# matwilso/generative_models

Hardware: AMD Instinct MI355X
Metric: ddpm_train_images_per_sec (higher is better)
Workload: dtype fp16_fwd+bf16_bwd; 1 GPU; DDPM train step, 3x32x32, SimpleUnet C=128, 2048 images per GPU, T=1000 (BASELINE.json configs[2]); key=cfg2, global_batch=2048, parallelism=dp1

## Files before the change

### generative_models_amd/diffusion/simple_unet.py

```python
import math
import os
from collections import OrderedDict

import torch
from torch import nn

from .. import ops

MAX_TIMESTEPS = 256


def _res_names(prefix, cin, cout, emb):
    out = [
        (f"{prefix}.in_layers.0.weight", (cin,)), (f"{prefix}.in_layers.0.bias", (cin,)),
        (f"{prefix}.in_layers.2.weight", (cout, cin, 3, 3)), (f"{prefix}.in_layers.2.bias", (cout,)),
        (f"{prefix}.emb_layers.1.weight", (cout, emb)), (f"{prefix}.emb_layers.1.bias", (cout,)),
        (f"{prefix}.out_layers.0.weight", (cout,)), (f"{prefix}.out_layers.0.bias", (cout,)),
        (f"{prefix}.out_layers.3.weight", (cout, cout, 3, 3)), (f"{prefix}.out_layers.3.bias", (cout,)),
    ]
    if cin != cout:
        out += [(f"{prefix}.skip_connection.weight", (cout, cin, 1, 1)), (f"{prefix}.skip_connection.bias", (cout,))]
    return out


# ... 608 lines not shown
                ds, dgp, dbp = ops.gn_silu_bwd(da, s, *gn[2:], dadd1=dskip, dadd2=add2, dxsum=ssum)
            if grads:
                ops.colsum(dgp, gw[i * C:(i + 1) * C], defer=True); ops.colsum(dbp, gb[i * C:(i + 1) * C], defer=True)
            outs.append((ds, ssum))
        return outs

    def prepare_forward(self, dev=None):
        if self._packs_stale or self._packed_version != self._version_sum():
            self._repack()
        dev = self.flat_params.device if dev is None else dev
        self._freq_table(MAX_TIMESTEPS, dev)
        self._freq_table(4, dev)

    def forward_hip(self, x, logsnr, guide=None, cond_w=None, ctx=None, want_nu=False):
        if want_nu and not self.learn_var:
            raise ValueError("forward_hip: want_nu on a network without the variance head (learn_var)")
        if self._packs_stale or self._packed_version != self._version_sum():
            self._repack()
        P, C, T = self._pv, self.channels, self.act_dtype
        B, cin, H, W = x.shape
        if cin != self.in_channels or H % 4 or W % 4:
            raise ValueError(f"input {tuple(x.shape)}: need {self.in_channels} channels and H, W divisible by 4")
        x = ops.aligned(x.float())
        logsnr, guide, cond_w = ops.aligned(logsnr), ops.aligned(guide), ops.aligned(cond_w)
        if ops.EMB_SIDE and ops.WGRAD_STREAM and x.is_cuda and not torch.cuda.is_current_stream_capturing():
            box = []
            self._on_side(lambda: box.append(self._embed_fwd(logsnr, guide, cond_w, ctx)), tuple(t for t in (logsnr, guide, cond_w) if t is not None))
            emb_all = box[0]
            self._emb_pending = emb_all
        else:
            emb_all = self._embed_fwd(logsnr, guide, cond_w, ctx)
        H2, W2, H4, W4 = H // 2, W // 2, H // 4, W // 4
        t0 = ops.stem_fwd(x, P["down.seq.0.conv.weight"], P["down.seq.0.conv.bias"], C, T)
        t1 = self._res_fwd("down.seq.1", [t0], emb_all, 0, ctx)
        t2 = self._res_fwd("down.seq.2", [t1], emb_all, 1, ctx)
        t3 = self._conv([t2], self._packs["down.seq.3.conv"][0], C, 3, ops.STRIDE2, (H2, W2),
                            bias=P["down.seq.3.conv.bias"])
        t4 = self._res_fwd("down.seq.4", [t3], emb_all, 2, ctx)
        t5 = self._res_fwd("down.seq.5", [t4], emb_all, 3, ctx)
        t6 = self._conv([t5], self._packs["down.seq.6.conv"][0], C, 3, ops.STRIDE2, (H4, W4),
                            bias=P["down.seq.6.conv.bias"])
        t7 = self._res_fwd("turn", [t6], emb_all, 4, ctx)
        if self.attention:
            t7 = self._attn_fwd(t7, ctx)
        u0r = self._res_fwd("up.seq.0.0", [t7, t6], emb_all, 5, ctx)
        u0 = self._upsample_conv("up.seq.0.1.conv", u0r, (H2, W2))
        u1 = self._res_fwd("up.seq.1", [u0, t5], emb_all, 6, ctx)
        u2 = self._res_fwd("up.seq.2", [u1, t4], emb_all, 7, ctx)
        u3r = self._res_fwd("up.seq.3.0", [u2, t3], emb_all, 8, ctx)
        u3 = self._upsample_conv("up.seq.3.1.conv", u3r, (H, W))
        u4 = self._res_fwd("up.seq.4", [u3, t2], emb_all, 9, ctx)
        u5 = self._res_fwd("up.seq.5", [u4, t1], emb_all, 10, ctx)
        u6 = self._res_fwd("up.seq.6", [u5, t0], emb_all, 11, ctx)
        ao, mo, ro = ops.gn_silu_fwd(u6, P["out.0.weight"], P["out.0.bias"], self._g1)
        out = ops.head_fwd(ao, P["out.2.weight"], P["out.2.bias"])
        if ctx is not None:
            ctx["net"] = (x, t2, t5, u0r, u3r, u6, ao, mo, ro)
            ctx["dims"] = (B, H, W)
        if want_nu:
            rows = B if want_nu is True else int(want_nu)
            if not 1 <= rows <= B:
                raise ValueError(f"forward_hip: want_nu = {want_nu} rows of a batch of {B}")
            return out, ops.head_fwd(ao if rows == B else ao[:rows], P["out_var.weight"], P["out_var.bias"])
        return out

    def grad_buckets(self):
        names = [n for n, _ in self._inventory]
        def rng(pred):
            return self.arena_range([n for n in names if pred(n)])
        late = ("up.seq.4", "up.seq.5", "up.seq.6", "out.", "out_var.")
        mid = ("up.seq.0", "up.seq.1", "up.seq.2", "up.seq.3")
        emb = ("time_embed", "cond_w_embed", "guide_embed")
        is_emb = lambda n: n.startswith(emb) or ".emb_layers." in n or n.endswith(".in_layers.2.bias")
        b0 = rng(lambda n: n.startswith(late) and not is_emb(n))
        b1 = rng(lambda n: n.startswith(mid) and not is_emb(n))
        b2 = rng(lambda n: (n.startswith("down.") or n.startswith("turn.") or n.startswith("attn.")) and not is_emb(n))
        b3 = rng(is_emb)
        buckets = [b0, b1, b2, b3]
        assert sorted(buckets)[0][0] == 0 and sorted(buckets)[-1][1] == self._arena_size
        srt = sorted(buckets)
        assert all(srt[i][1] == srt[i + 1][0] for i in range(3)), "gradient buckets must tile the arena"
        return buckets

    def backward_hip(self, ctx, dout, on_grads_ready=None, join_side_before_ready=True, want_dx=False, dnu=None):
        if ops.WGRAD_CUS > 0 and ops.WGRAD_STREAM and dout.is_cuda and self._cu_part is None and not (
                torch.distributed.is_available() and torch.distributed.is_initialized() and torch.distributed.get_world_size() > 1):
            full = ops.get_cu_limit()
            self._cu_part = (full, min(ops.WGRAD_CUS, full - 8))
            ops.set_cu_limit(full - self._cu_part[1])
            try:
                return self.backward_hip(ctx, dout, on_grads_ready, join_side_before_ready, want_dx, dnu)
            finally:
                ops.set_cu_limit(full)
                self._cu_part = None
        if dnu is not None and not self.learn_var:
            raise ValueError("backward_hip: dnu on a network without the variance head (learn_var)")
        if dnu is not None and tuple(dnu.shape) != tuple(dout.shape):
            raise ValueError(f"backward_hip: dnu has shape {tuple(dnu.shape)}, dout {tuple(dout.shape)}")
        join = self._join_side if (on_grads_ready is not None and join_side_before_ready) else None
        dt0 = self._backward_schedule(ctx, ops.aligned(dout.float()), True, on_grads_ready, join,
                                      dnu=None if dnu is None else ops.aligned(dnu.float()))
        return ops.stem_dgrad(dt0, self._pv["down.seq.0.conv.weight"]) if want_dx else None

    def input_vjp_hip(self, ctx, r):
        x = ctx["net"][0]
        if tuple(r.shape) != tuple(x.shape):
            raise ValueError(f"input_vjp_hip: r has shape {tuple(r.shape)}, the network output {tuple(x.shape)}")
        dt0 = self._backward_schedule(ctx, ops.aligned(r.float()), False)
        return ops.stem_dgrad(dt0, self._pv["down.seq.0.conv.weight"])

    def _backward_schedule(self, ctx, dout, grads, ready=None, join=None, dnu=None):
        P, G, C, T = self._pv, self._gv, self.channels, self.compute_dtype
        B, H, W = ctx["dims"]
        H2, W2 = H // 2, W // 2
        x, t2, t5, u0r, u3r, u6, ao, mo, ro = ctx["net"]
        dev = dout.device
        demb_all = torch.empty((B, 12 * C), device=dev, dtype=torch.float32) if grads else None
        pair = grads and ready is None
        ready = ready if ready is not None else (lambda k: None)
        join = join if join is not None else (lambda: None)
        res = lambda name, d, dsum, blk, extra=None, defer=False: self._res_bwd(name, ctx, d, dsum, demb_all, blk, extra_add=extra, grads=grads,
                                                                               defer_skip=defer and pair)

        def bucket_done(k):
            if grads:
                ops.flush_colsums(); join()
                ready(k)

        def up(name, d, dsum, src):
            if grads:
                ops.colsum(dsum, G[name + ".bias"], defer=True)
                self._upsample_wgrad(name, d, src)
            dsrc = self._upsample_dgrad(name, d)
            return dsrc, (ops.chansum(dsrc) if grads else None)

        def down(name, d, dsum, src, hw, skip):
            if grads:
                ops.colsum(dsum, G[name + ".bias"], defer=True)
                self._wgrad(d, [src], 3, ops.STRIDE2, G[name + ".weight"])
            dsrc = self._conv([d], self._packs[name][1], C, 3, ops.TRANSPOSED2, hw, residual=skip)
            return dsrc, (ops.chansum(dsrc) if grads else None)

        if grads:
            o = self._offsets["out.2.weight"]
            nhead = self.in_channels * C * 9
            assert self._offsets["out.2.bias"] == o + (nhead + 3) // 4 * 4 == o + nhead
            self._on_side(lambda: ops.head_wgrad(dout, ao, self.flat_grads[o:o + nhead + self.in_channels]), (dout, ao))
        dao = ops.head_dgrad(dout, P["out.2.weight"], T)
        if dnu is None and grads and self.learn_var:
            self.flat_grads[self._offsets["out_var.weight"]:].zero_()
        if dnu is not None:
            if grads:
                ov = self._offsets["out_var.weight"]
                assert self._offsets["out_var.bias"] == ov + nhead
                self._on_side(lambda: ops.head_wgrad(dnu, ao, self.flat_grads[ov:ov + nhead + self.in_channels]), (dnu, ao))
            ops.add_into(dao, ops.head_dgrad(dnu, P["out_var.weight"], T))
        s6 = torch.empty((B, C), device=dev, dtype=torch.float32) if grads else None
        du6, dgp, dbp = ops.gn_silu_bwd(dao, u6, P["out.0.weight"], P["out.0.bias"], mo, ro, dxsum=s6)
        if grads:
            ops.colsum(dgp, G["out.0.weight"], defer=True); ops.colsum(dbp, G["out.0.bias"], defer=True)

        (du5, s5), (dt0a, _) = res("up.seq.6", du6, s6, 11, defer=True)
        (du4, s4), (dt1a, _) = res("up.seq.5", du5, s5, 10, defer=True)
        (du3, s3), (dt2a, _) = res("up.seq.4", du4, s4, 9)
        bucket_done(0)
        du3r, s3r = up("up.seq.3.1.conv", du3, s3, u3r)
        (du2, s2), (dt3a, _) = res("up.seq.3.0", du3r, s3r, 8, defer=True)
        (du1, s1), (dt4a, _) = res("up.seq.2", du2, s2, 7, defer=True)
        (du0, s0), (dt5a, _) = res("up.seq.1", du1, s1, 6)
        du0r, s0r = up("up.seq.0.1.conv", du0, s0, u0r)
        (dt7, s7), (dt6a, _) = res("up.seq.0.0", du0r, s0r, 5)
        if self.attention:
            dt7, s7 = self._attn_bwd(ctx, dt7, grads=grads)
        bucket_done(1)
        ((dt6, s6t),) = res("turn", dt7, s7, 4, [dt6a])
        dt5, s5t = down("down.seq.6.conv", dt6, s6t, t5, (H2, W2), dt5a)
        ((dt4, s4t),) = res("down.seq.5", dt5, s5t, 3, [dt4a])
        ((dt3, s3t),) = res("down.seq.4", dt4, s4t, 2, [dt3a])
        dt2, s2t = down("down.seq.3.conv", dt3, s3t, t2, (H, W), dt2a)
        ((dt1, s1t),) = res("down.seq.2", dt2, s2t, 1, [dt1a])
        ((dt0, s0t),) = res("down.seq.1", dt1, s1t, 0, [dt0a])
        if grads:
            ops.colsum(s0t, G["down.seq.0.conv.bias"], defer=True)
            self._on_side(lambda: ops.stem_wgrad(x, dt0, G["down.seq.0.conv.weight"]), (x, dt0))
            bucket_done(2)
            self._embed_bwd(ctx, demb_all)
            ops.flush_colsums()
            ready(3)
            self._join_side()
        return dt0

    def zero_grad_arena(self):
        self.flat_grads.zero_()

    def forward(self, x, timesteps, guide=None, cond_w=None, want_nu=False):
        if torch.is_grad_enabled() and (x.requires_grad or any(p.requires_grad for p in self.parameters())):
            if want_nu:
                return SimpleUnetVarFunction.apply(self, x, timesteps, guide, cond_w, *self.parameters())
            return SimpleUnetFunction.apply(self, x, timesteps, guide, cond_w, *self.parameters())
        return self.forward_hip(x, timesteps, guide, cond_w, want_nu=bool(want_nu))
# ... 45 lines not shown
```

### generative_models_amd/ops.py

```python
import functools
import math

import os

import torch

from ._lib import C, K, check, kernel_name, lib

F32, BF16, F16 = C["GMK_F32"], C["GMK_BF16"], C["GMK_F16"]
_DT = {torch.float32: F32, torch.bfloat16: BF16, torch.float16: F16}
_HALF = (torch.bfloat16, torch.float16)
NORMAL, STRIDE2, UPSAMPLE2, TRANSPOSED2 = C["GMK_CONV_NORMAL"], C["GMK_CONV_STRIDE2"], C["GMK_CONV_UPSAMPLE2"], C["GMK_CONV_TRANSPOSED2"]

PROFILE = None


def instantiation_key(name, dtype):
    if dtype not in _HALF:
        return None
    t = "f16" if dtype == torch.float16 else "bf16"
    if name == "conv3x3_halo_ws_kernel":
        return f"{name}<{t}>"
    if name == "conv3x3_halo_ws_kernel[+1x1 skip]":
        return f"conv3x3_halo_ws_kernel<{t},+skip>"
# ... 84 lines not shown

def aligned(t):
    if t is None:
        return None
    t = t.contiguous()
    return t.clone() if t.data_ptr() % 16 else t


def _f32(t, name):
    return _chk(t, torch.float32, name)


def check_stream(seed, offset):
    seed, offset = int(seed), int(offset)
    if not (0 <= seed < 1 << 64 and 0 <= offset < 1 << 64):
        raise ValueError(f"offset = {offset}, seed = {seed}: Philox counters and seeds are unsigned 64-bit")
    return seed, offset


def pack_conv_weight(w, w_fwd, w_dgrad):
    _f32(w, "w")
    cout, cin, k, _ = w.shape
    ref = w_fwd if w_fwd is not None else w_dgrad
    for t in (w_fwd, w_dgrad):
        if t is not None:
            _chk(t, name="pack")
            assert t.numel() == w.numel()
    if w_fwd is not None and w_dgrad is not None and w_fwd.dtype != w_dgrad.dtype:
        pack_conv_weight(w, w_fwd, None)
        pack_conv_weight(w, None, w_dgrad)
        return
    check(lib.gmk_pack_conv_weight(_p(w), _p(w_fwd), _p(w_dgrad), cout, cin, k, _DT[ref.dtype], _s()), "pack_conv_weight")


def pack_conv_weights_multi(arena, packs, table, fwd_f16=None):
    import ctypes
    _f32(arena, "arena"); _chk(packs, name="packs")
    n = len(table[0])
    arrs = [(ctypes.c_int * n)(*[int(v) for v in col]) for col in table]
    flags = (ctypes.c_int * n)(*[int(v) for v in fwd_f16]) if fwd_f16 is not None else None
    check(lib.gmk_pack_conv_weights_multi(_p(arena), _p(packs), n, *arrs, flags, _DT[packs.dtype], _s()), "pack_conv_weights_multi")


GN_STATS = False
GN_FUSE = os.environ.get("GMK_GN_FUSE", "1") != "0"
GN_FUSE_MIN_HW = int(os.environ.get("GMK_GN_FUSE_MIN_HW", "2048"))
SKIP_FOLD = os.environ.get("GMK_SKIP_FOLD", "1") != "0"
SKIP_FOLD_OVER_FUSE = os.environ.get("GMK_SKIP_FOLD_FUSE", "fold") != "fuse"
EMB_SIDE = os.environ.get("GMK_EMB_SIDE", "1") == "1"
FWD_SIDE = os.environ.get("GMK_FWD_SIDE", "0") == "1"
WGRAD_CUS = int(os.environ.get("GMK_WGRAD_CUS", "0"))
WGRAD_STREAM = os.environ.get("GMK_WGRAD_STREAM", "1") != "0"
GN_PAIR = os.environ.get("GMK_GN_PAIR", "1") != "0"


def _xadd_stride(xadd, B, C):
    if xadd is None:
        return 0
    assert xadd.dtype == torch.float32 and xadd.shape == (B, C) and xadd.stride(1) == 1 and xadd.is_cuda
    return xadd.stride(0)


def gn_silu_fwd(x, gamma, beta, groups, eps=1e-5, dropout=None, xadd=None):
    _chk(x, name="x"); _f32(gamma, "gamma"); _f32(beta, "beta")
    B, H, W, C = x.shape
    assert gamma.numel() == C and beta.numel() == C
    y = torch.empty_like(x)
    ncol = groups if groups > 0 else (C - groups - 1) // -groups
    mean = torch.empty((B, ncol), device=x.device, dtype=torch.float32)
    rstd = torch.empty_like(mean)
    mean._gn_groups = groups
    st = getattr(x, "_gn_stats", None)
    part, tp, nt = st if st is not None else (None, 0, 0)
    dp, dseed, doff = dropout if dropout is not None else (0.0, 0, 0)
    xs = _xadd_stride(xadd, B, C)
    with _Timed("gn_silu_fwd", 0.0, _nbytes(x, y)):
        check(lib.gmk_gn_silu_fwd(_p(x), _p(y), _p(gamma), _p(beta), _p(mean), _p(rstd), B, H * W, C, groups, eps, _p(part), tp, nt,
                                  float(dp), int(dseed), int(doff), _p(xadd), xs, _DT[x.dtype], _s()), "gn_silu_fwd")
    return y, mean, rstd


def gn_stats(x, gamma, beta, groups, tab_scale, tab_shift, eps=1e-5, xadd=None):
    _chk(x, name="x"); _f32(gamma, "gamma"); _f32(beta, "beta")
    assert x.dtype in _HALF
    B, H, W, C = x.shape
    for t in (tab_scale, tab_shift):
        assert t.dtype == torch.float32 and t.shape == (B, C) and t.stride(1) == 1 and t.is_cuda and t.data_ptr() % 16 == 0
    assert tab_scale.stride(0) == tab_shift.stride(0)
    mean = torch.empty((B, groups), device=x.device, dtype=torch.float32)
    rstd = torch.empty_like(mean)
    xs = _xadd_stride(xadd, B, C)
    with _Timed("gn_stats", 0.0, _nbytes(x)):
        check(lib.gmk_gn_stats(_p(x), _p(gamma), _p(beta), _p(mean), _p(rstd), _p(tab_scale), _p(tab_shift), tab_scale.stride(0), B, H * W, C,
                               groups, eps, _p(xadd), xs, _DT[x.dtype], _s()), "gn_stats")
    return mean, rstd


def conv_gn_fusable(srcs, cout=128):
    s0 = srcs[0]
    c1 = srcs[1].shape[3] if len(srcs) > 1 else 0
    B, H, W, c0 = s0.shape
    return s0.dtype in _HALF and H * W >= GN_FUSE_MIN_HW and bool(lib.gmk_conv_gn_fusable(B, H, W, c0, c1, cout))


def gn_silu_bwd(dy, x, gamma, beta, mean, rstd, dadd1=None, dadd2=None, dxsum=None, dropout=None, xadd=None):
    _chk(x, name="x"); _chk(dy, name="dy")
# ... 329 lines not shown
    B, cin, H, W = x.shape
    assert w.shape == (C, cin, 3, 3)
    y = torch.empty((B, H, W, C), device=x.device, dtype=dtype)
    with _Timed("stem_fwd", 2.0 * B * H * W * C * cin * 9, _nbytes(x, y)):
        check(lib.gmk_stem_fwd(_p(x), _p(w), _p(bias), _p(y), B, cin, H, W, C, _DT[dtype], _s()), "stem_fwd")
    return y


def stem_wgrad(x, dy, dw):
    _f32(x, "x"); _chk(dy, name="dy")
    B, cin, H, W = x.shape
    C = dy.shape[3]
    nb = lib.gmk_stem_wgrad_blocks(B * H * W)
    part = torch.empty((nb, C * cin * 9), device=x.device, dtype=torch.float32)
    with _Timed("stem_wgrad", 2.0 * B * H * W * C * cin * 9, _nbytes(x, dy)):
        check(lib.gmk_stem_wgrad(_p(x), _p(dy), _p(part), B, cin, H, W, C, _DT[dy.dtype], _s()), "stem_wgrad")
    return colsum(part, dw)


def head_fwd(a, w, bias):
    _chk(a, name="a"); _f32(w, "w"); _f32(bias, "bias")
    B, H, W, C = a.shape
    cout = w.shape[0]
    assert w.shape == (cout, C, 3, 3)
    out = torch.empty((B, cout, H, W), device=a.device, dtype=torch.float32)
    with _Timed("head_fwd", 2.0 * B * H * W * C * cout * 9, _nbytes(a, out)):
        check(lib.gmk_head_fwd(_p(a), _p(w), _p(bias), _p(out), B, cout, H, W, C, _DT[a.dtype], _s()), "head_fwd")
    return out


def head_dgrad(dout, w, dtype):
    _f32(dout, "dout"); _f32(w, "w")
    B, cout, H, W = dout.shape
    C = w.shape[1]
    da = torch.empty((B, H, W, C), device=dout.device, dtype=dtype)
    with _Timed("head_dgrad", 2.0 * B * H * W * C * cout * 9, _nbytes(dout, da)):
        check(lib.gmk_head_dgrad(_p(dout), _p(w), _p(da), B, cout, H, W, C, _DT[dtype], _s()), "head_dgrad")
    return da


def head_wgrad(dout, a, dwb):
    _f32(dout, "dout"); _chk(a, name="a")
    B, cout, H, W = dout.shape
    C = a.shape[3]
    n = cout * C * 9 + cout
    assert dwb.numel() == n
    nb = lib.gmk_head_wgrad_blocks(B * H * W)
    part = torch.empty((nb, n), device=a.device, dtype=torch.float32)
    with _Timed("head_wgrad", 2.0 * B * H * W * C * cout * 9, _nbytes(dout, a)):
        check(lib.gmk_head_wgrad(_p(dout), _p(a), _p(part), B, cout, H, W, C, _DT[a.dtype], _s()), "head_wgrad")
    return colsum(part, dwb)


def add_into(a, b):
    _chk(a, name="a"); _chk(b, a.dtype, "b")
    if a.shape != b.shape or a.numel() % 8 or a.dtype not in (torch.float32, torch.bfloat16):
        raise ValueError(f"add_into: shapes {tuple(a.shape)} and {tuple(b.shape)} of {a.dtype}: one shape, a multiple of 8 elements, fp32 or bf16")
    check(lib.gmk_add_into(_p(a), _p(b), a.numel(), _DT[a.dtype], _s()), "add_into")
    return a


def stem_dgrad(dy, w):
    if dy.dim() != 4 or w.dim() != 4 or tuple(w.shape[2:]) != (3, 3) or w.shape[0] != dy.shape[3]:
        raise ValueError(f"stem_dgrad: bad shapes dy {tuple(dy.shape)} and w {tuple(w.shape)}: expected [B, H, W, C] and [C, cin, 3, 3]")
    if dy.dtype not in _DT:
        raise ValueError(f"stem_dgrad: dy dtype {dy.dtype}")
    _f32(w, "w"); _chk(dy, name="dy")
    B, H, W, C = dy.shape
    cin = w.shape[1]
    dx = torch.empty((B, cin, H, W), device=dy.device, dtype=torch.float32)
    with _Timed("stem_dgrad", 2.0 * B * H * W * C * cin * 9, _nbytes(dy, dx)):
        check(lib.gmk_stem_dgrad(_p(dy), _p(w), _p(dx), B, cin, H, W, C, _DT[dy.dtype], _s()), "stem_dgrad")
    return dx


def timestep_freqs(max_period, device):
    half = 32
    return torch.exp(-math.log(max_period) * torch.arange(0, half, dtype=torch.float32) / half).to(device)


def timestep_embedding(t, freqs):
    _f32(t, "t"); _f32(freqs, "freqs")
    B = t.numel()
    out = torch.empty((B, 64), device=t.device, dtype=torch.float32)
    check(lib.gmk_timestep_embedding(_p(t), _p(freqs), _p(out), B, _s()), "timestep_embedding")
    return out


def guide_onehot(guide):
    _chk(guide, torch.int64, "guide")
    B = guide.numel()
    onehot = torch.empty((B, 10), device=guide.device, dtype=torch.float32)
    keep = torch.empty((B,), device=guide.device, dtype=torch.float32)
    check(lib.gmk_guide_onehot(_p(guide), _p(onehot), _p(keep), B, _s()), "guide_onehot")
    return onehot, keep


def label_drop(y, p, seed, offset):
    seed, offset = check_stream(seed, offset)
    _chk(y, torch.int64, "y")
    check(lib.gmk_label_drop(_p(y), y.numel(), float(p), seed, offset, _s()), "label_drop")
    return y


def batch_gather(images, labels, index, *, pad, binarize, flip_p=0.0, seed=0, offset=0, trusted=False):
    seed, offset = check_stream(seed, offset)
# ... 923 lines not shown
```

### include/gmk.h

```cpp
#ifndef GMK_H
#define GMK_H
#include <stdint.h>

#ifdef __cplusplus
extern "C" {
#endif

#define GMK_F32 0
#define GMK_BF16 1
#define GMK_F16 2
#define GMK_ERR_ARG (-1)

#define GMK_CONV_NORMAL 0
#define GMK_CONV_STRIDE2 1
#define GMK_CONV_UPSAMPLE2 2
#define GMK_CONV_TRANSPOSED2 3

int gmk_version(void);
const char* gmk_last_error(void);
#define GMK_KERNEL_TABLE(X)                                                                                                               \
    X(CONV_IGEMM, 1, "conv_igemm_kernel")                                                                                                 \
    X(CONV_IGEMM_DMA, 2, "conv_igemm_dma_kernel")                                                                                         \
    X(CONV_HALO, 3, "conv3x3_halo_kernel")                                                                                                \
    X(CONV_HALO_WS, 4, "conv3x3_halo_ws_kernel")                                                                                          \
// ... 70 lines not shown
                         const void* dy_dn, const void* dadd_dn, const float* gamma_dn, const float* beta_dn, const float* mean_dn,
                         const float* rstd_dn, float* dgamma_part_dn, float* dbeta_part_dn, int groups_dn, void* dx, float* dxsum,
                         int dxsum_stride, int B, int HW, int C, const float* xadd, int xadd_stride, int x_dtype, void* stream);
int gmk_cast16(const void* src, void* dst, int64_t n, int src_dtype, int dst_dtype, void* stream);
int gmk_chansum(const void* x, float* out, int out_stride, int B, int HW, int C, int dtype, void* stream);
int gmk_colsum(const float* part, int64_t stride, float* out, int R, int C, int accumulate, void* stream);
int gmk_colsum_multi(int n, const float* const* part, const int64_t* stride, float* const* out, const int* R,
                     const int* C, void* stream);
int gmk_sumpool2x2(const void* x, void* y, int B, int H, int W, int C, int dtype, void* stream);

int gmk_conv_igemm(const void* src0, const void* src1, int c0, int c1, int B, int hs, int ws, int ho, int wo,
                   int ksize, int mode, const void* w, int w_rows, int n0, int cout, const float* bias,
                   const float* emb, int emb_stride, const void* residual, void* out, int out_cstride,
                   float* gn_stats, int64_t gn_stats_bytes, const float* gn_scale, const float* gn_shift, int gn_stride,
                   int dtype, void* stream);
int gmk_conv_gn_fusable(int B, int H, int W, int c0, int c1, int cout);
int gmk_conv1x1_pair(const void* src, int c, int B, int H, int W, const void* w, int w_rows, int n0, void* out_a, void* out_b,
                     int dtype, void* stream);
int gmk_conv3x3_skipfold_ok(int B, int H, int W, int c0, int cs, int cout);
int gmk_conv3x3_skipfold(const void* src, int c0, int B, int H, int W, const void* w, int w_rows, int n0, int cout,
                         const float* bias, const void* sk0, const void* sk1, int cs, const void* wsk, int wsk_rows, int nsk0,
                         const float* bias_sk, void* out, int out_cstride, int dtype, void* stream);
#define GMK_SUBPIXEL_UPSAMPLE 0
#define GMK_SUBPIXEL_TRANSPOSED 1
#define GMK_SUBPIXEL_UPSAMPLE_DGRAD 2
int gmk_conv_subpixel_ok(int B, int H, int W, int cin, int cout, int dtype);
int gmk_pack_upsample_weight(const float* w, void* w_sub, void* w_sub_dgrad, int cout, int cin, int dtype, int dgrad_dtype, void* stream);
int gmk_conv_subpixel(const void* src, int B, int H, int W, int cin, const void* w, int w_rows, int n0, int cout, int mode,
                      const float* bias, const void* residual, void* out, int out_cstride, int dtype, void* stream);
int gmk_conv_wgrad_subpixel_ok(int B, int H, int W, int cin, int cout);
int64_t gmk_conv_wgrad_subpixel_workspace_bytes(int B, int H, int W, int cin, int cout);
int gmk_conv_wgrad_subpixel(const void* dy, int dy_cstride, const void* x, int B, int H, int W, int cin, int cout, float* dw,
                            void* workspace, int64_t workspace_bytes, int dtype, int x_dtype, void* stream);
int gmk_gn_stats(const void* x, const float* gamma, const float* beta, float* mean, float* rstd, float* tab_scale,
                 float* tab_shift, int tab_stride, int B, int HW, int C, int groups, float eps, const float* xadd,
                 int xadd_stride, int dtype, void* stream);
int gmk_conv_wgrad(const void* dy, int dy_cstride, const void* src0, const void* src1, int c0, int c1, int B,
                   int hs, int ws, int ho, int wo, int ksize, int mode, float* dw, int cout, void* workspace,
                   int64_t workspace_bytes, int dtype, int x_dtype, void* stream);

int gmk_stem_fwd(const float* x, const float* w, const float* bias, void* y, int B, int cin, int H, int W, int C,
                 int dtype, void* stream);
int gmk_stem_wgrad_blocks(int64_t n_pixels);
int gmk_stem_wgrad(const float* x, const void* dy, float* dw_part, int B, int cin, int H, int W, int C, int dtype,
                   void* stream);
int gmk_head_fwd(const void* a, const float* w, const float* bias, float* out, int B, int cout, int H, int W, int C,
                 int dtype, void* stream);
int gmk_head_dgrad(const float* dout, const float* w, void* da, int B, int cout, int H, int W, int C, int dtype,
                   void* stream);
int gmk_head_wgrad_blocks(int64_t n_pixels);
int gmk_head_wgrad(const float* dout, const void* a, float* dw_part, int B, int cout, int H, int W, int C, int dtype,
                   void* stream);
int gmk_stem_dgrad(const void* dy, const float* w, float* dx, int B, int cin, int H, int W, int C, int dtype, void* stream);

int gmk_timestep_embedding(const float* t, const float* freqs, float* out, int B, void* stream);
int gmk_guide_onehot(const int64_t* guide, float* onehot, float* keep, int B, void* stream);
int gmk_label_drop(int64_t* y, int B, float p, uint64_t seed, uint64_t offset, void* stream);
int gmk_batch_gather(const uint8_t* images, const uint8_t* labels, const int64_t* index, int B, int64_t N, int C, int H, int W, int pad,
                     int binarize, float flip_p, uint64_t seed, uint64_t offset, float* x, int64_t* y, void* stream);
int gmk_to_uint8(const float* x, uint8_t* out, int64_t n_images, int C, int H, int W, int crop, void* stream);
int gmk_image_grid(const float* x, uint8_t* out, int T, int N, int C, int H, int W, int crop, int ncol, int gap, int fill, int out_channels,
                   int row_prefix, void* stream);
int gmk_mean(const float* x, int n, float* out, void* stream);
int gmk_gemm_f32(const float* A, int64_t sa0, int64_t sa1, const float* B, int64_t sb0, int64_t sb1, float* C,
                 int64_t ldc, int M, int N, int K, const float* bias, const float* bias2, const float* rowscale,
                 int silu, int accumulate, void* workspace, int64_t workspace_bytes, void* stream);
int64_t gmk_gemm_f32_workspace_bytes(int M, int N, int K);
int gmk_silu_bwd(const float* dpost, const float* pre, const float* rowscale, float* dpre, int64_t n, int ncols,
                 void* stream);
int gmk_scale_rows(const float* in, const float* rowscale, float* out, int64_t n, int ncols, void* stream);

int gmk_rng_normal(float* out, int64_t n, uint64_t seed, uint64_t offset, void* stream);
int gmk_rng_uniform(float* out, int64_t n, uint64_t seed, uint64_t offset, void* stream);
int gmk_q_sample(const float* x, const float* eps, const float* u, float* logsnr, float* z, int B, int64_t n,
                 void* stream);
#define GMK_SCHED_COSINE 0
#define GMK_SCHED_UNIFORM 1
#define GMK_SCHED_BETA_CONST 2
#define GMK_SCHED_BETA_LINEAR 3
int gmk_q_sample_sched(const float* x, const float* eps, const float* u, float* logsnr, float* z, int B, int64_t n, int kind, float a,
                       float b, float lmin, float lmax, float shift, void* stream);
#define GMK_MEAN_V 0
#define GMK_MEAN_EPS 1
#define GMK_MEAN_X 2
int gmk_v_loss(const float* v, const float* z, const float* x, const float* eps, const float* logsnr, float* loss_b,
               float* x_mse, float* eps_mse, float* dv, float grad_scale, int loss_type, int mean_type, int B, int64_t n,
               void* stream);
#define GMK_LOSS_W_SNR_PLUS1 0
#define GMK_LOSS_W_MIN_SNR 1
#define GMK_X_LOSS_KEEP 12288
int gmk_x_loss_w(const float* v, const float* z, const float* x, const float* logsnr, float* loss_b, float* x_mse, float* dv,
                 float grad_scale, int weight_type, float gamma, int mean_type, int B, int64_t n, void* stream);
int gmk_u_stratified(const float* u0, float* u, int B, void* stream);
#define GMK_PROFILE_BINS 64
int gmk_loss_profile(const float* u, const float* v0, const float* v1, int B, float decay, float* state, void* stream);
int gmk_u_importance(const float* state, const float* u0, float* u, float* w, int B, float warm, float floor, float* p_out, float* w_out,
                     void* stream);
int gmk_sampler_step(const float* v, const float* v_uncond, const float* cond_w, const float* z, const float* noise,
                     float logsnr_t, float logsnr_s, int is_last, float* z_next, float* x_pred, float* eps_pred,
                     float* z_dup, float* logsnr_next, int mean_type, int B, int64_t n, void* stream);
int gmk_dpm_solver_step(const float* v, const float* v_uncond, const float* cond_w, const float* z, float* x_hist, float logsnr_t,
                        float logsnr_s, float coef_z, float coef_x, float coef_prev, int is_last, float* z_next, float* x_pred,
                        float* eps_pred, float* z_dup, float* logsnr_next, int mean_type, int B, int64_t n, void* stream);
#define GMK_DYN_THRESHOLD_KEYS 12288
int gmk_dyn_threshold(const float* v, const float* v_uncond, const float* cond_w, const float* z, float logsnr_t, int k_lo, float frac,
                      float* s_out, float* q_out, int mean_type, int B, int64_t n, void* stream);
// ... 105 lines not shown
```

Baseline: 46820 images/s.

## Fuse output GroupNorm-SiLU with head conv and recompute activation in head wgrad

Adds a single forward kernel that computes GroupNorm statistics, applies SiLU and runs the 3x3 head convolution from LDS, so the normalized activation is never written to global memory. The kernel saves per-sample scale and shift tables. A new head weight-gradient kernel rebuilds the activation from the raw input and those tables while tiling. The aim is to remove a full-resolution 128-channel activation round trip through memory and one kernel launch. The cost is recomputing the activation in backward and more complex kernels that only handle 32x32 or 28x28 shapes without learned variance.

```diff
diff --git a/generative_models_amd/csrc/out_block.hip b/generative_models_amd/csrc/out_block.hip
--- /dev/null
+++ b/generative_models_amd/csrc/out_block.hip
@@ -0,0 +1,402 @@
+#include "conv_plan.h"
+#include "gmk_common.h"
+
+namespace {
+
+typedef __attribute__((ext_vector_type(4))) unsigned int u32x4_t;
+constexpr int kC = 128, kG = 32;
+constexpr int kRing = 16;
+constexpr int kStageRow = 144;
+constexpr int kStageWave = 32 * kStageRow;
+constexpr int kMaxWaves = 16;
+constexpr int kTapBytes = 27 * kRing * 32 * 4;
+constexpr int kOutFwdLds = kMaxWaves * kStageWave + kTapBytes + 2 * 2 * 4 * 64 * 16;
+
+__device__ __forceinline__ void lds_barrier() {
+    asm volatile("s_waitcnt lgkmcnt(0)" ::: "memory");
+    __builtin_amdgcn_s_barrier();
+}
+
+template <typename T>
+__device__ __forceinline__ void unpack8(const u32x4_t r, float (&v)[8]) {
+#pragma unroll
+    for (int k = 0; k < 4; ++k) unpack_pair<T>(r[k], v[2 * k], v[2 * k + 1]);
+}
+
+template <typename T, int ITER>
+__global__ __launch_bounds__(1024) void out_fwd_kernel(const T* __restrict__ x, T* __restrict__ y, const float* __restrict__ gamma,
+                                                       const float* __restrict__ beta, const float* __restrict__ w,
+                                                       const float* __restrict__ bias, float* __restrict__ out, float* __restrict__ mean,
+                                                       float* __restrict__ rstd, float* __restrict__ tab_sc, float* __restrict__ tab_sh,
+                                                       int tab_stride, int W, int cs, float eps, unsigned x_bytes, int B) {
+    extern __shared__ __attribute__((aligned(16))) char smem[];
+    __shared__ float red[kMaxWaves][8][4];
+    __shared__ float smean[kG], srstd[kG];
+    constexpr int H = 2 * ITER, NG = (ITER + 3) / 4;
+    const int tid = threadIdx.x, lane = tid & 63, wave = tid >> 6;
+    const int wph = blockDim.x >> 7;
+    const int half = wave >= wph ? 1 : 0, ws = wave - half * wph;
+    const int tl = ws * 64 + lane, vec = tl & 7, pl = tl >> 3;
+    const int planes = 2 * W, HW = H * W, K = 9 * cs;
+    const int c0 = half * 64;
+    const __amdgpu_buffer_rsrc_t rsx = __builtin_amdgcn_make_buffer_rsrc(const_cast<T*>(x), 0, (int)x_bytes, 0x00020000);
+    const __amdgpu_buffer_rsrc_t rsy = __builtin_amdgcn_make_buffer_rsrc(y, 0, y ? (int)x_bytes : 0, 0x00020000);
+    const unsigned toff = (unsigned)(pl * kC + c0 + vec * 8) * 2u, sbytes = (unsigned)HW * (kC * 2u), sstride = (unsigned)planes * (kC * 2u);
+    u32x4_t raw[ITER];
+#pragma unroll
+    for (int i = 0; i < ITER; ++i) raw[i] = __builtin_amdgcn_raw_buffer_load_b128(rsx, toff, blockIdx.x * sbytes + i * sstride, 0);
+    typedef typename Frag16<T>::type frag_t;
+    const int r = lane & 31, h = lane >> 5;
+    frag_t* wl = reinterpret_cast<frag_t*>(smem + kMaxWaves * kStageWave + kTapBytes) + half * 512 + lane;
+    if (ws == 0) {
+        const int sj = r / 9, tj = r - sj * 9;
+#pragma unroll
+        for (int ks = 0; ks < 4; ++ks) {
+            frag_t whi, wlo;
+#pragma unroll
+            for (int e = 0; e < 8; ++e) {
+                const int c = c0 + 16 * ks + 8 * h + e;
+                const float wv = r >= K ? 0.f : w[((size_t)sj * kC + c) * 9 + tj];
+                const T hi = (T)wv;
+                whi[e] = hi;
+                wlo[e] = (T)(wv - (float)hi);
+            }
+            wl[ks * 64] = whi;
+            wl[256 + ks * 64] = wlo;
+        }
+    }
+    float* tapl = reinterpret_cast<float*>(smem + kMaxWaves * kStageWave);
+    for (int b = blockIdx.x; b < B; b += (int)gridDim.x) {
+        const int nb = b + (int)gridDim.x;
+        const unsigned soff = (unsigned)b * sbytes;
+        int t = tid;
+        asm volatile("" : "+v"(t));
+        const int lane = t & 63, wave = t >> 6;
+        const int half = wave >= wph ? 1 : 0, ws = wave - half * wph;
+        const int tl = ws * 64 + lane, vec = tl & 7, pl = tl >> 3, c0 = half * 64;
+        const int r = lane & 31, h = lane >> 5;
+        const frag_t* wl = reinterpret_cast<const frag_t*>(smem + kMaxWaves * kStageWave + kTapBytes) + half * 512 + lane;
+        char* stage = smem + wave * kStageWave;
+        const int jj = lane >> 3;
+        const int plq = ws * 8 + (r & 7);
+        const int qy = plq >= W ? 1 : 0, qx = plq - qy * W;
+        float s0 = 0.f, q0 = 0.f, s1 = 0.f, q1 = 0.f;
+#pragma unroll
+        for (int i = 0; i < ITER; ++i) {
+            asm volatile("" : "+v"(raw[i]), "+v"(s0), "+v"(q0), "+v"(s1), "+v"(q1));
+            float v[8];
+            unpack8<T>(raw[i], v);
+            s0 += (v[0] + v[1]) + (v[2] + v[3]);
+            q0 += (v[0] * v[0] + v[1] * v[1]) + (v[2] * v[2] + v[3] * v[3]);
+            s1 += (v[4] + v[5]) + (v[6] + v[7]);
+            q1 += (v[4] * v[4] + v[5] * v[5]) + (v[6] * v[6] + v[7] * v[7]);
+        }
+#pragma unroll
+        for (int i = 0; i < ITER; ++i) asm volatile("" : "+v"(raw[i]));
+        s0 = lanes_sum_from<8>(s0); q0 = lanes_sum_from<8>(q0); s1 = lanes_sum_from<8>(s1); q1 = lanes_sum_from<8>(q1);
+        if (lane < 8) { red[wave][lane][0] = s0; red[wave][lane][1] = q0; red[wave][lane][2] = s1; red[wave][lane][3] = q1; }
+        __syncthreads();
+        if (t < kG) {
+            const int hh = t >> 4, hv = t & 15, vv = hv >> 1, hf = hv & 1;
+            float s = 0.f, q = 0.f;
+            for (int wv = hh * wph; wv < hh * wph + wph; ++wv) { s += red[wv][vv][hf * 2]; q += red[wv][vv][hf * 2 + 1]; }
+            const float n = 4.0f * (float)HW;
+            const float m = s / n;
+            const float var = fmaxf(q / n - m * m, 0.f);
+            const float r = 1.0f / sqrtf(var + eps);
+            smean[t] = m; srstd[t] = r;
+            mean[b * kG + t] = m; rstd[b * kG + t] = r;
+        }
+        __syncthreads();
+        float sc[8], sh[8];
+#pragma unroll
+        for (int i = 0; i < 8; ++i) {
+            const int cl = vec * 8 + i, g = half * 16 + (cl >> 2), c = c0 + cl;
+            sc[i] = srstd[g] * gamma[c];
+            sh[i] = beta[c] - (smean[g] - 0.f) * sc[i];
+        }
+        if (pl == 0) {
+#pragma unroll
+            for (int i = 0; i < 8; ++i) {
+                tab_sc[(size_t)b * tab_stride + c0 + vec * 8 + i] = sc[i];
+                tab_sh[(size_t)b * tab_stride + c0 + vec * 8 + i] = sh[i];
+            }
+        }
+#pragma unroll
+        for (int g = 0; g < NG; ++g) {
+#pragma unroll
+            for (int ii = 0; ii < 4; ++ii) {
+                const int i = 4 * g + ii;
+                if (i >= ITER) continue;
+                asm volatile("" : "+v"(raw[i]));
+                float v[8];
+                unpack8<T>(raw[i], v);
+#pragma unroll
+                for (int k = 0; k < 8; ++k) v[k] = siluf_(fmaf(v[k], sc[k], sh[k]));
+                u32x4_t yv;
+#pragma unroll
+                for (int k = 0; k < 4; ++k) yv[k] = pack_pair<T>(v[2 * k], v[2 * k + 1]);
+                if (y) __builtin_amdgcn_raw_buffer_store_b128(yv, rsy, toff, soff + i * sstride, 0);
+                *reinterpret_cast<u32x4_t*>(stage + (ii * 8 + jj) * kStageRow + vec * 16) = yv;
+            }
+            lds_barrier();
+            const int qi = 4 * g + (r >> 3);
+            const bool qok = qi < ITER;
+            float* tq = tapl + ((2 * qi + qy) & (kRing - 1)) * 32 + qx;
+#pragma unroll
+            for (int phase = 0; phase < 2; ++phase) {
+                if (half == phase) {
+                    f32x16 acc;
+#pragma unroll
+                    for (int e = 0; e < 16; ++e) {
+                        const int j = (e & 3) + 8 * (e >> 2) + 4 * h;
+                        acc[e] = (phase == 1 && qok && j < K) ? tq[j * kRing * 32] : 0.f;
+                    }
+#pragma unroll
+                    for (int ks = 0; ks < 4; ++ks) {
+                        const frag_t bv = *reinterpret_cast<const frag_t*>(stage + r * kStageRow + (2 * ks + h) * 16);
+                        acc = mfma_32x32x16<T>(wl[ks * 64], bv, acc);
+                        acc = mfma_32x32x16<T>(wl[256 + ks * 64], bv, acc);
+                    }
+                    if (qok) {
+#pragma unroll
+                        for (int e = 0; e < 16; ++e) {
+                            const int j = (e & 3) + 8 * (e >> 2) + 4 * h;
+                            if (j < K) tq[j * kRing * 32] = acc[e];
+                        }
+                    }
+                }
+                lds_barrier();
+            }
+            if (nb < B) {
+#pragma unroll
+                for (int ii = 0; ii < 4; ++ii)
+                    if (4 * g + ii < ITER) raw[4 * g + ii] = __builtin_amdgcn_raw_buffer_load_b128(rsx, toff, (unsigned)nb * sbytes + (4 * g + ii) * sstride, 0);
+            }
+            const int lo = g == 0 ? 0 : 8 * g - 1, hi = g == NG - 1 ? H : 8 * g + 7;
+            const int per = (hi - lo) * W;
+            for (int o = t; o < cs * per; o += (int)blockDim.x) {
+                const int s = o / per, rem = o - s * per;
+                const int oyl = rem / W, ox = rem - oyl * W, oy = lo + oyl;
+                float sum = bias[s];
+#pragma unroll
+                for (int ky = 0; ky < 3; ++ky) {
+                    const int iy = oy + ky - 1;
+#pragma unroll
+                    for (int kx = 0; kx < 3; ++kx) {
+                        const int ix = ox + kx - 1;
+                        if ((unsigned)iy < (unsigned)H && (unsigned)ix < (unsigned)W)
+                            sum += tapl[((s * 9 + ky * 3 + kx) * kRing + (iy & (kRing - 1))) * 32 + ix];
+                    }
+                }
+                out[((size_t)(b * cs + s) * H + oy) * W + ox] = sum;
+            }
+        }
+    }
+}
+
+constexpr int kTileWin = 128 + 2 * 128 + 2;
+
+template <typename T, int CSN>
+__global__ __launch_bounds__(256, 2) void wgrad3x3_tile16_gn_kernel(const float* __restrict__ small, const T* __restrict__ big,
+                                                                   const float* __restrict__ tab_sc, const float* __restrict__ tab_sh,
+                                                                   int tab_stride, float* __restrict__ part, int H, int W, int C,
+                                                                   int tiles_per_sample, unsigned ntiles, unsigned small_bytes,
+                                                                   unsigned big_bytes) {
+    static_assert(sizeof(T) == 2, "16-bit tensors only");
+    constexpr int K = 9 * CSN, kRow = 272;
+    constexpr unsigned kBadOff = 0xFFFFFF00u;
+    typedef bf16x8 frag_t;
+    typedef __attribute__((ext_vector_type(4))) unsigned int u32x4s;
+    __shared__ __attribute__((aligned(16))) char smem[4 * 128 * 32 * 4];
+    __shared__ float bred[4][4][2];
+    char* bigt = smem;
+    float* win = reinterpret_cast<float*>(smem + 128 * kRow);
+    static_assert(128 * kRow + 3 * kTileWin * 4 <= (int)sizeof(smem), "tile + window fit the reduction buffer");
+    const int tid = threadIdx.x, lane = tid & 63, wave = tid >> 6;
+    const int r = lane & 31, h = lane >> 5;
+    const int HW = H * W, WIN = 128 + 2 * W + 2;
+    const __amdgpu_buffer_rsrc_t rss = __builtin_amdgcn_make_buffer_rsrc(const_cast<float*>(small), 0, (int)small_bytes, 0x00020000);
+    const __amdgpu_buffer_rsrc_t rsb = __builtin_amdgcn_make_buffer_rsrc(const_cast<T*>(big), 0, (int)big_bytes, 0x00020000);
+    const bool kin = r < K;
+    const int s_ = kin ? r / 9 : 0, t = kin ? r % 9 : 4;
+    const int dy = 1 - t / 3, dx = 1 - t % 3;
+    const int woff = s_ * kTileWin + dy * W + dx + (W + 1);
+    float bsum = 0.f;
+    f32x16 acc[4];
+#pragma unroll
+    for (int cb = 0; cb < 4; ++cb)
+#pragma unroll
+        for (int e = 0; e < 16; ++e) acc[cb][e] = 0.f;
+
+    struct Tile { u32x4s br[8]; float wr[CSN][2]; f32x4 sc[2], sh[2]; unsigned rows; };
+    auto load_tile = [&](unsigned tile, Tile& tl) {
+        const bool on = tile < ntiles;
+        const int b = on ? (int)(tile / (unsigned)tiles_per_sample) : 0, pp0 = on ? ((int)tile - b * tiles_per_sample) * 128 : 0;
+        tl.rows = 0;
+#pragma unroll
+        for (int i = 0; i < 8; ++i) {
+            const int c = tid + 256 * i, row = c >> 4;
+            const bool in = on && pp0 + row < HW;
+            tl.rows |= (unsigned)in << i;
+            tl.br[i] = __builtin_amdgcn_raw_buffer_load_b128(rsb, in ? (unsigned)(b * HW + pp0) * 256u + (unsigned)c * 16u : kBadOff, 0, 0);
+        }
+        const float* ts = tab_sc + (size_t)b * tab_stride + (tid & 15) * 8;
+        const float* th = tab_sh + (size_t)b * tab_stride + (tid & 15) * 8;
+        tl.sc[0] = *reinterpret_cast<const f32x4*>(ts); tl.sc[1] = *reinterpret_cast<const f32x4*>(ts + 4);
+        tl.sh[0] = *reinterpret_cast<const f32x4*>(th); tl.sh[1] = *reinterpret_cast<const f32x4*>(th + 4);
+#pragma unroll
+        for (int j = 0; j < 2; ++j) {
+            const int i = tid + 256 * j, flat = pp0 - (W + 1) + i;
+            const bool ok = on && i < WIN && flat >= 0 && flat < HW;
+#pragma unroll
+            for (int sc = 0; sc < CSN; ++sc)
+                tl.wr[sc][j] = __builtin_bit_cast(float, __builtin_amdgcn_raw_buffer_load_b32(rss, ok ? (unsigned)((b * CSN + sc) * HW + flat) * 4u : kBadOff, 0, 0));
+        }
+    };
+    auto park_tile = [&](const Tile& tl) {
+#pragma unroll
+        for (int i = 0; i < 8; ++i) {
+            const int c = tid + 256 * i;
+            float v[8];
+            unpack8<T>(tl.br[i], v);
+            u32x4s a;
+#pragma unroll
+            for (int k = 0; k < 4; ++k) {
+                const float lo = siluf_(fmaf(v[2 * k], tl.sc[k >> 1][(2 * k) & 3], tl.sh[k >> 1][(2 * k) & 3]));
+                const float hi = siluf_(fmaf(v[2 * k + 1], tl.sc[k >> 1][(2 * k + 1) & 3], tl.sh[k >> 1][(2 * k + 1) & 3]));
+                a[k] = (tl.rows >> i) & 1u ? pack_pair<T>(lo, hi) : 0u;
+            }
+            *reinterpret_cast<u32x4s*>(bigt + (c >> 4) * kRow + (c & 15) * 16) = a;
+        }
+#pragma unroll
+        for (int j = 0; j < 2; ++j) {
+            const int i = tid + 256 * j;
+            if (i < WIN) {
+#pragma unroll
+                for (int sc = 0; sc < CSN; ++sc) win[sc * kTileWin + i] = tl.wr[sc][j];
+            }
+        }
+    };
+    Tile tl;
+    load_tile(blockIdx.x, tl);
+    for (unsigned tile = blockIdx.x; tile < ntiles; tile += gridDim.x) {
+        __syncthreads();
+        park_tile(tl);
+        __syncthreads();
+        load_tile(tile + gridDim.x, tl);
+        const int pp0 = (int)(tile % (unsigned)tiles_per_sample) * 128;
+#pragma unroll
+        for (int ks = 0; ks < 2; ++ks) {
+            const int pl = wave * 32 + 16 * ks + 8 * h;
+            int pp = pp0 + pl;
+            int y = pp / W, x = pp - y * W;
+            frag_t bhi, blo;
+#pragma unroll
+            for (int e = 0; e < 8; ++e) {
+                const int ok = (int)kin & (int)(pp < HW) & (int)((unsigned)(y + dy) < (unsigned)H) & (int)((unsigned)(x + dx) < (unsigned)W);
+                float v = win[woff + pl + e];
+                v = ok ? v : 0.f;
+                bsum += t == 4 ? v : 0.f;
+                const bf16_t hi = (bf16_t)v;
+                bhi[e] = hi;
+                blo[e] = (bf16_t)(v - (float)hi);
+                ++pp; ++x;
+                const int wrap = x >= W;
+                x = wrap ? 0 : x; y += wrap;
+            }
+#pragma unroll
+            for (int cb = 0; cb < 4; ++cb) {
+                frag_t a, alo;
+#pragma unroll
+                for (int e = 0; e < 8; ++e) {
+                    const T av = *reinterpret_cast<const T*>(bigt + (pl + e) * kRow + (cb * 32 + r) * 2);
+                    if constexpr (__is_same(T, bf16_t)) a[e] = av;
+                    else {
+                        const float af = (float)av;
+                        const bf16_t hi = (bf16_t)af;
+                        a[e] = hi;
+                        alo[e] = (bf16_t)(af - (float)hi);
+                    }
+                }
+                if constexpr (!__is_same(T, bf16_t)) acc[cb] = __builtin_amdgcn_mfma_f32_32x32x16_bf16(alo, bhi, acc[cb], 0, 0, 0);
+                acc[cb] = __builtin_amdgcn_mfma_f32_32x32x16_bf16(a, blo, acc[cb], 0, 0, 0);
+                acc[cb] = __builtin_amdgcn_mfma_f32_32x32x16_bf16(a, bhi, acc[cb], 0, 0, 0);
+            }
+        }
+    }
+    __syncthreads();
+    float* red = reinterpret_cast<float*>(smem);
+#pragma unroll
+    for (int cb = 0; cb < 4; ++cb)
+#pragma unroll
+        for (int e = 0; e < 16; ++e) red[wave * (128 * 32) + (cb * 32 + (e & 3) + 8 * (e >> 2) + 4 * h) * 32 + r] = acc[cb][e];
+    if (kin && t == 4) bred[wave][s_][h] = bsum;
+    __syncthreads();
+    const size_t rowlen = (size_t)CSN * C * 9 + CSN;
+    float* out = part + (size_t)blockIdx.x * rowlen;
+    for (int idx = tid; idx < CSN * 128 * 9; idx += 256) {
+        const int sc = idx / (128 * 9), rem = idx - sc * 128 * 9, c = rem / 9, j = sc * 9 + (rem - c * 9);
+        out[idx] = (red[c * 32 + j] + red[128 * 32 + c * 32 + j]) + (red[2 * 128 * 32 + c * 32 + j] + red[3 * 128 * 32 + c * 32 + j]);
+    }
+    if (tid < CSN) {
+        float sum = 0.f;
+#pragma unroll
+        for (int wv = 0; wv < 4; ++wv) sum += bred[wv][tid][0] + bred[wv][tid][1];
+        out[(size_t)CSN * C * 9 + tid] = sum;
+    }
+}
+
+int out_iter(int H, int W) { return H == 32 && W == 32 ? 16 : H == 28 && W == 28 ? 14 : 0; }
+
+}
+
+extern "C" int gmk_out_fuse_ok(int B, int cout, int H, int W, int C, int groups, int dtype) {
+    SmallPlan p;
+    return B > 0 && cout >= 1 && cout <= 3 && C == kC && groups == kG && gmk_is16(dtype) && out_iter(H, W) > 0 &&
+           (int64_t)B * H * W < (1ll << 24) && (int64_t)B * H * W * kC * 2 < 0xFFFFFF00ll && gmk_kernel_choice(2, "GMK_GN_KERNEL") == 0 &&
+           gmk_kernel_choice(3, "GMK_DEV_VARIANT") == 0 && gmk_wgrad3_plan(B, cout, H, W, C, dtype, 0, gmk_cu_limit(), &p) &&
+           p.kernel == GMK_K_WGRAD3_TILE16;
+}
+
+extern "C" int gmk_out_fwd(const void* x, const float* gamma, const float* beta, const float* w, const float* bias, float* out, void* y,
+                           float* mean, float* rstd, float* tab_scale, float* tab_shift, int tab_stride, int B, int cout, int H, int W, int C,
+                           int groups, float eps, int dtype, void* stream) {
+    GMK_REQUIRE(x && gamma && beta && w && bias && out && mean && rstd && tab_scale && tab_shift, "gmk_out_fwd: null pointer");
+    GMK_REQUIRE(gmk_out_fuse_ok(B, cout, H, W, C, groups, dtype), "gmk_out_fwd: unsupported shape B=%d cout=%d %dx%d C=%d G=%d dtype=%d", B, cout,
+                H, W, C, groups, dtype);
+    GMK_REQUIRE(tab_stride >= C, "gmk_out_fwd: tab_stride %d < C %d", tab_stride, C);
+    const unsigned threads = (unsigned)(W / 4) * 128u, lds = kOutFwdLds, grid = (unsigned)(B < gmk_cu_limit() ? B : gmk_cu_limit());
+    hipStream_t s = gmk_stream(stream);
+    gmk_with_type<f16_t, bf16_t>(dtype, [&](auto tag) {
+        using T = typename decltype(tag)::type;
+        auto launch = [&](auto kernel) {
+            [[maybe_unused]] static const hipError_t attr = hipFuncSetAttribute((const void*)kernel, hipFuncAttributeMaxDynamicSharedMemorySize, kOutFwdLds);
+            kernel<<<grid, threads, lds, s>>>((const T*)x, (T*)y, gamma, beta, w, bias, out, mean, rstd, tab_scale, tab_shift, tab_stride, W, cout, eps,
+                                           (unsigned)((size_t)B * H * W * kC * 2), B);
+        };
+        if (out_iter(H, W) == 16) launch(out_fwd_kernel<T, 16>);
+        else launch(out_fwd_kernel<T, 14>);
+    });
+    return gmk_check_launch("gmk_out_fwd");
+}
+
+extern "C" int gmk_head_wgrad_gn(const float* dout, const void* x, const float* tab_scale, const float* tab_shift, int tab_stride,
+                                 float* dw_part, int B, int cout, int H, int W, int C, int dtype, void* stream) {
+    SmallPlan p;
+    GMK_REQUIRE(dout && x && tab_scale && tab_shift && dw_part, "gmk_head_wgrad_gn: null pointer");
+    GMK_REQUIRE(tab_stride >= C && tab_stride % 4 == 0 && (uintptr_t)tab_scale % 16 == 0 && (uintptr_t)tab_shift % 16 == 0,
+                "gmk_head_wgrad_gn: the tables are 16-byte aligned rows of >= C floats (stride %d)", tab_stride);
+    GMK_REQUIRE(gmk_is16(dtype) && cout <= 3 && gmk_wgrad3_plan(B, cout, H, W, C, dtype, 0, gmk_cu_limit(), &p) && p.kernel == GMK_K_WGRAD3_TILE16,
+                "gmk_head_wgrad_gn: unsupported shape B=%d cout=%d %dx%d C=%d dtype=%d", B, cout, H, W, C, dtype);
+    const unsigned npix = (unsigned)(B * H * W), small_bytes = npix * cout * 4, big_bytes = (unsigned)((size_t)npix * C * 2);
+    hipStream_t s = gmk_stream(stream);
+    gmk_with_type<f16_t, bf16_t>(dtype, [&](auto tag) {
+        using T = typename decltype(tag)::type;
+        gmk_with_count<3, 2, 1>(cout, [&](auto n) {
+            wgrad3x3_tile16_gn_kernel<T, decltype(n)::value><<<p.grid, p.block, 0, s>>>(dout, (const T*)x, tab_scale, tab_shift, tab_stride, dw_part, H,
+                                                                                       W, C, p.tps, p.ntiles, small_bytes, big_bytes);
+        });
+    });
+    return gmk_check_launch("gmk_head_wgrad_gn");
+}
diff --git a/generative_models_amd/diffusion/simple_unet.py b/generative_models_amd/diffusion/simple_unet.py
--- a/generative_models_amd/diffusion/simple_unet.py
+++ b/generative_models_amd/diffusion/simple_unet.py
@@ -684,8 +684,12 @@
         u4 = self._res_fwd("up.seq.4", [u3, t2], emb_all, 9, ctx)
         u5 = self._res_fwd("up.seq.5", [u4, t1], emb_all, 10, ctx)
         u6 = self._res_fwd("up.seq.6", [u5, t0], emb_all, 11, ctx)
-        ao, mo, ro = ops.gn_silu_fwd(u6, P["out.0.weight"], P["out.0.bias"], self._g1)
-        out = ops.head_fwd(ao, P["out.2.weight"], P["out.2.bias"])
+        if not self.learn_var and ops.out_fuse_ok(u6, self._g1, self.in_channels):
+            out, mo, ro, tsc, tsh, _ = ops.out_fwd(u6, P["out.0.weight"], P["out.0.bias"], self._g1, P["out.2.weight"], P["out.2.bias"])
+            ao = (tsc, tsh)
+        else:
+            ao, mo, ro = ops.gn_silu_fwd(u6, P["out.0.weight"], P["out.0.bias"], self._g1)
+            out = ops.head_fwd(ao, P["out.2.weight"], P["out.2.bias"])
         if ctx is not None:
             ctx["net"] = (x, t2, t5, u0r, u3r, u6, ao, mo, ro)
             ctx["dims"] = (B, H, W)
@@ -777,7 +781,10 @@
             o = self._offsets["out.2.weight"]
             nhead = self.in_channels * C * 9
             assert self._offsets["out.2.bias"] == o + (nhead + 3) // 4 * 4 == o + nhead
-            self._on_side(lambda: ops.head_wgrad(dout, ao, self.flat_grads[o:o + nhead + self.in_channels]), (dout, ao))
+            if isinstance(ao, tuple):
+                self._on_side(lambda: ops.head_wgrad_gn(dout, u6, ao[0], ao[1], self.flat_grads[o:o + nhead + self.in_channels]), (dout, u6, ao[0], ao[1]))
+            else:
+                self._on_side(lambda: ops.head_wgrad(dout, ao, self.flat_grads[o:o + nhead + self.in_channels]), (dout, ao))
         dao = ops.head_dgrad(dout, P["out.2.weight"], T)
         if dnu is None and grads and self.learn_var:
             self.flat_grads[self._offsets["out_var.weight"]:].zero_()
diff --git a/generative_models_amd/ops.py b/generative_models_amd/ops.py
--- a/generative_models_amd/ops.py
+++ b/generative_models_amd/ops.py
@@ -160,6 +160,7 @@
 WGRAD_CUS = int(os.environ.get("GMK_WGRAD_CUS", "0"))
 WGRAD_STREAM = os.environ.get("GMK_WGRAD_STREAM", "1") != "0"
 GN_PAIR = os.environ.get("GMK_GN_PAIR", "1") != "0"
+OUT_FUSE = os.environ.get("GMK_OUT_FUSE", "1") != "0"
 
 
 def _xadd_stride(xadd, B, C):
@@ -595,6 +596,51 @@
     return colsum(part, dwb)
 
 
+def out_fuse_ok(x, groups, cout):
+    if not OUT_FUSE or x.dtype not in _HALF or x.dim() != 4:
+        return False
+    B, H, W, C = x.shape
+    return bool(lib.gmk_out_fuse_ok(B, cout, H, W, C, groups, _DT[x.dtype]))
+
+
+def out_fwd(x, gamma, beta, groups, w, bias, eps=1e-5, want_y=False):
+    _chk(x, name="x"); _f32(gamma, "gamma"); _f32(beta, "beta"); _f32(w, "w"); _f32(bias, "bias")
+    B, H, W, C = x.shape
+    cout = w.shape[0]
+    assert w.shape == (cout, C, 3, 3) and bias.numel() == cout and gamma.numel() == C and beta.numel() == C
+    if not out_fuse_ok(x, groups, cout):
+        raise ValueError(f"out_fwd: x {tuple(x.shape)} of {x.dtype}, {groups} groups, {cout} image channels is no shape of the fused out block")
+    out = torch.empty((B, cout, H, W), device=x.device, dtype=torch.float32)
+    mean = torch.empty((B, groups), device=x.device, dtype=torch.float32)
+    rstd = torch.empty_like(mean)
+    mean._gn_groups = groups
+    tabs = torch.empty((2, B, C), device=x.device, dtype=torch.float32)
+    y = torch.empty_like(x) if want_y else None
+    with _Timed("out_fwd_kernel", 2.0 * B * H * W * C * cout * 9, _nbytes(x, out, y), fixed=True):
+        check(lib.gmk_out_fwd(_p(x), _p(gamma), _p(beta), _p(w), _p(bias), _p(out), _p(y), _p(mean), _p(rstd), _p(tabs[0]), _p(tabs[1]), C,
+                              B, cout, H, W, C, groups, eps, _DT[x.dtype], _s()), "out_fwd")
+    return out, mean, rstd, tabs[0], tabs[1], y
+
+
+def head_wgrad_gn(dout, x, tab_scale, tab_shift, dwb):
+    _f32(dout, "dout"); _chk(x, name="x")
+    assert x.dtype in _HALF
+    B, cout, H, W = dout.shape
+    C = x.shape[3]
+    assert x.shape == (B, H, W, C)
+    for t in (tab_scale, tab_shift):
+        assert t.dtype == torch.float32 and t.shape == (B, C) and t.stride(1) == 1 and t.is_cuda and t.data_ptr() % 16 == 0
+    assert tab_scale.stride(0) == tab_shift.stride(0)
+    n = cout * C * 9 + cout
+    assert dwb.numel() == n
+    nb = lib.gmk_head_wgrad_blocks(B * H * W)
+    part = torch.empty((nb, n), device=x.device, dtype=torch.float32)
+    with _Timed("wgrad3x3_tile16_gn_kernel", 2.0 * B * H * W * C * cout * 9, _nbytes(dout, x), fixed=True):
+        check(lib.gmk_head_wgrad_gn(_p(dout), _p(x), _p(tab_scale), _p(tab_shift), tab_scale.stride(0), _p(part), B, cout, H, W, C,
+                                    _DT[x.dtype], _s()), "head_wgrad_gn")
+    return colsum(part, dwb)
+
+
 def add_into(a, b):
     _chk(a, name="a"); _chk(b, a.dtype, "b")
     if a.shape != b.shape or a.numel() % 8 or a.dtype not in (torch.float32, torch.bfloat16):
diff --git a/include/gmk.h b/include/gmk.h
--- a/include/gmk.h
+++ b/include/gmk.h
@@ -146,6 +146,12 @@
 int gmk_head_wgrad(const float* dout, const void* a, float* dw_part, int B, int cout, int H, int W, int C, int dtype,
                    void* stream);
 int gmk_stem_dgrad(const void* dy, const float* w, float* dx, int B, int cin, int H, int W, int C, int dtype, void* stream);
+int gmk_out_fuse_ok(int B, int cout, int H, int W, int C, int groups, int dtype);
+int gmk_out_fwd(const void* x, const float* gamma, const float* beta, const float* w, const float* bias, float* out, void* y,
+                float* mean, float* rstd, float* tab_scale, float* tab_shift, int tab_stride, int B, int cout, int H, int W, int C,
+                int groups, float eps, int dtype, void* stream);
+int gmk_head_wgrad_gn(const float* dout, const void* x, const float* tab_scale, const float* tab_shift, int tab_stride,
+                      float* dw_part, int B, int cout, int H, int W, int C, int dtype, void* stream);
 
 int gmk_timestep_embedding(const float* t, const float* freqs, float* out, int B, void* stream);
 int gmk_guide_onehot(const int64_t* guide, float* onehot, float* keep, int B, void* stream);
```

Measured after the change: 46890 images/s (median of 6 runs). No clear change (+0.2%).
